# CederGroupHub/sparse-lm

Hardware: AMD Instinct MI355X
Metric: fits/sec over 50-alpha Lasso path at n=100k p=5k (higher is better)
Workload: dtype f64

## Files before the change

### include/slm_engine.h

```cpp
#ifndef SLM_ENGINE_H
#define SLM_ENGINE_H

#include <stddef.h>
#include <stdint.h>

#ifdef __cplusplus
extern "C" {
#endif

#define SLM_ABI_VERSION 24

typedef enum slm_status {
  SLM_OK = 0,
  SLM_ERR_BAD_ARG = 1,
  SLM_ERR_OOM = 2,
  SLM_ERR_HIP = 3,
  SLM_ERR_NO_DEVICE = 4,
  SLM_ERR_COMM = 5,
  SLM_ERR_NOT_CONVERGED = 6,
  SLM_ERR_NON_FINITE = 7,
  SLM_ERR_UNSUPPORTED = 8
} slm_status;

typedef struct slm_engine slm_engine;
// ... 36 lines not shown
  int32_t route;
  int32_t n_lanes;
  int32_t lane_out;
  int32_t probe_lanes;
  int32_t xtr_only;
} slm_gradient_opts;
int slm_gradient_ex(slm_dataset* ds, const double* z, const slm_gradient_opts* opts, double* g_out, double* loss_out,
                    int32_t reps, double* ms_out);

int slm_gradient_lanes(slm_dataset* ds, int32_t route, int32_t n_lanes, const double* Z, const double* row_weights,
                       const double* n_eff, const int32_t* cov_index, int64_t n_rows, double* G_out, double* loss_out,
                       char* kernels_out, int32_t kernels_len);

#define SLM_WSL_GATHER_X 1u
#define SLM_WSL_XTY 2u
typedef struct slm_ws_lanes_opts {
  int32_t route;
  int32_t n_lanes;
  const double* Z;
  const int32_t* on_ws;
  const double* row_weights;
  const double* n_eff;
  const int32_t* cov_index;
  const int32_t* cols;
  const int32_t* k_end;
  int32_t n_builds;
  uint32_t flags;
} slm_ws_lanes_opts;
int slm_working_set_lanes(slm_dataset* ds, const slm_ws_lanes_opts* opts, double* G_out, double* loss_out, int32_t* set_of_out,
                          int32_t* n_sets_out, double* gram_out, double* xw_out, double* xty_out, char* kernels_out,
// ... 262 lines not shown
```

### sparse-lm_amd/csrc/engine_internal.hpp

```cpp
#pragma once
#include <hip/hip_runtime.h>

#include <dlfcn.h>
#include <stdarg.h>
#include <stdio.h>
#include <stdlib.h>
#include <string.h>

#include <algorithm>
#include <cmath>
#include <chrono>
#include <condition_variable>
#include <memory>
#include <mutex>
#include <numeric>
#include <string>
#include <vector>

#include "../../include/slm_engine.h"
#include "host_logic.hpp"
#include "data_kernels.hpp"
#include "grad_kernel.hpp"
#include "tail_kernels.hpp"
#include "ws_kernels.hpp"
// ... 280 lines not shown
int enqueue_gradient_split(const slm_host::Knobs& kn, slm_dataset* ds, const LaneSetup& ls, const double* y, const int* done, const PathCtl* ctl, const WsArgs* wa,
                           hipEvent_t ev_start, hipEvent_t ev_stop, int64_t n_rows = 0, bool unit_bracket = false, const int* skip = nullptr,
                           GradNames* names = nullptr);
bool split_usable(const slm_host::Knobs& kn, slm_dataset* ds);
int ensure_xt(const slm_host::Knobs& kn, slm_dataset* ds);
int ensure_x32s(slm_dataset* ds, int64_t n_rows, bool* usable);
void x32_drop(slm_dataset* ds);
int enqueue_sample_f32(slm_dataset* ds, int64_t n_rows, double n_eff, int n_lanes, const int* done, bool* queued);
int check_launch();
void launch_rowdot(const slm_host::Knobs& kn, slm_dataset* ds, const SplitKernel* sk, int nblk, int B, SplitArgs& a, hipStream_t s,
                  const char** name = nullptr);
int enqueue_gradient_cov(slm_dataset* ds, int B, const int* entry_of, const int* done, hipEvent_t ev_start, hipEvent_t ev_stop,
                         const PathCtl* ctl = nullptr, const WsArgs* wa = nullptr, GradNames* names = nullptr);
void launch_tail(const TailArgs& ta, hipStream_t s);
int64_t sketch_rows(int64_t n);
int power_iteration(const slm_host::Knobs& kn, slm_dataset* ds, const LaneSetup& ls_in, double* L_out , int iters, int64_t n_rows = 0);
int estimate_lipschitz(const slm_host::Knobs& kn, slm_dataset* ds, double* L_out, int iters);
int allow_big_lds(const void* fn, int device);
static const int kProfStride = 3;
static const int kPowerItersSolve = 2;
int cov_fingerprints(slm_dataset* ds, const double* const* w, int count, double* out );
int cov_find(const slm_dataset* ds, double fp1, double fp2, double n_eff);
void cov_pending_drop(slm_dataset* ds);
int set_singleton_groups(slm_dataset* ds);
static const int kMgEntries = 8;
bool mg_possible(const slm_host::Knobs& kn, const slm_dataset* ds);
int mg_ensure(const slm_host::Knobs& kn, slm_dataset* ds, const double* w, double n_eff, bool own, double fp1, double fp2, int* entry_out);
void mg_invalidate(slm_dataset* ds);
void mg_free(slm_dataset* ds);
int mg_enqueue_round(slm_dataset* ds, const TailArgs& ta, int n_lanes, int inner_iters, const int* done, int n_sets, const int* entry_of_set,
                     const int* set_of);
// ... 1 lines not shown
```

### sparse-lm_amd/csrc/engine_path.hip

```cpp
#include "engine_internal.hpp"
#include "ws_solve_kernels.hpp"

static int ws_policy(const slm_host::Knobs& kn, const slm_dataset* ds, uint32_t flags) {
  if (ds->max_group > WS_KCAP / 2 || ds->n < 4) return 0;
  if (kn.ws == 0 || (flags & SLM_FLAG_NO_WORKING_SET)) return 0;
  const bool big = (double)ds->n * (double)ds->ld >= 67108864.0;
  return (big || (flags & SLM_FLAG_WORKING_SET) || kn.ws == 1) ? 2 : 1;
}

static bool small_ok(const slm_host::Knobs& kn, const slm_dataset* ds, uint32_t flags) {
  if (!(flags & SLM_FLAG_ON_CHIP)) return false;
  if (flags & (SLM_FLAG_NO_RESTART | SLM_FLAG_PROFILE | SLM_FLAG_FISTA_ONLY | SLM_FLAG_WORKING_SET | SLM_FLAG_NO_WORKING_SET))
    return false;
  if (!kn.on_chip) return false;
  return ds->p <= SM_PMAX && (double)ds->n * (double)ds->ld <= 131072.0 && !row_sharded(ds);
}
static bool split_possible(const slm_dataset* ds) {
  return ds->sk != nullptr && (ds->sk->rowdot != nullptr || !ds->XT_failed);
}
static int max_lanes_for(const slm_host::Knobs& kn, const slm_dataset* ds, uint32_t flags) {
  if (small_ok(kn, ds, flags)) return ds->lane_cap;
  if ((ws_policy(kn, ds, flags) == 2 || (double)ds->n * (double)ds->ld >= 67108864.0) && split_possible(ds)) {
    if (ws_policy(kn, ds, flags) == 2 && !row_sharded(ds) && ds->sk->rowdot != nullptr && !ds->XT_failed)
      return kMaxLanes;
// ... 294 lines not shown
      const int l = first_lane[u];
      const double ne = ls.n_eff[l] > 0 ? ls.n_eff[l] : (double)ds->n_global;
      entry_of_set[u] = cov_find(ds, fp[2 * u], fp[2 * u + 1], ne);
      cov_on = entry_of_set[u] >= 0;
    }
    if (cov_on) {
      for (int l = 0; l < B; ++l) cov_entry[l] = entry_of_set[uniq_of[l]];
      if (!ds->cov_Z) SLM_TRY(dalloc(&ds->cov_Z, (size_t)ld * SPLIT_RSTRIDE * SPLIT_HALVES));
    }
  }
  return SLM_OK;
}

int PathCall::kept_sketch() {
  if (ds->sketch_valid && !(o.flags & SLM_FLAG_FRESH_L)) return SLM_OK;
  SLM_TRY(power_iteration(kn, ds, default_lanes(ds, 1), nullptr, slm_host::kSketchPowerIters, sketch_rows(ds->n)));
  HIP_TRY(hipMemcpyAsync(ds->lambda + ds->lane_cap, ds->lambda, sizeof(double), hipMemcpyDeviceToDevice, eng->stream));
  ds->sketch_valid = true;
  return SLM_OK;
}

int PathCall::seed_lipschitz() {
  for (int l = 0; l < kMaxCells; ++l) L_factor[l] = 1.0;
  if (o.L > 0.0 || small) {
    for (int l = 0; l < B; ++l) L[l] = o.L > 0.0 ? o.L : 1.0;
  } else {
    const auto t0 = std::chrono::steady_clock::now();
    bool ran = false;
    const bool sketch = ws_policy(kn, ds, o.flags) == 2 && n >= 65536;
    if (sketch && !(ds->L_valid && !(o.flags & SLM_FLAG_FRESH_L) && !any_rw && !custom_scale)) {
      const bool per_lane = any_rw || custom_scale;
      bool bounded = per_lane && !sharded;
// ... 489 lines not shown
  if (shared_path && interleave && mg_handover) hipLaunchKernelGGL(tail_handover_kernel, dim3(1), dim3(64), 0, s, ta);
  else if (shared_path && interleave && use_ws && !ws_late && !sharded && planned_end > 0 && kn.lag_handover)
    hipLaunchKernelGGL(lag_handover_kernel, dim3(1), dim3(64), 0, s, ta, &ds->ws_ctl->builds, &ds->ws_ctl->stale, (int)(planned_end - enq - 1));
  if (sharded) {
    if (use_ws && wa.Gx) {
      hipLaunchKernelGGL(stop_pack_kernel, dim3(1), dim3(64), 0, s, ta.gdone, ds->ctl, B,
                         wa.Gx + (size_t)wa.n_sets * WS_KCAP * WS_KCAP);
    } else {
      hipLaunchKernelGGL(stop_pack_kernel, dim3(1), dim3(64), 0, s, ta.gdone, ds->ctl, B, ds->stop_words);
      if (ws_comm_rc == 0) ws_comm_rc = all_reduce_sum(eng, ds->stop_words, STOP_WORDS);
      hipLaunchKernelGGL(stop_apply_kernel, dim3(1), dim3(64), 0, s, ta.gdone, ds->stop_words);
    }
  }
}

struct WsNames {
  const char* k[8];
  int n = 0;
  void add(const char* name) { if (n < 8) k[n++] = name; }
};
static void ws_enqueue_build(slm_dataset* ds, const WsArgs& wa, const CovSets* cs, bool xty, const int* done, int n_lanes, hipStream_t s,
                             WsNames* names = nullptr) {
  const int64_t n = ds->n;
  if (cs) {
    hipLaunchKernelGGL(ws_gram_cov_kernel, dim3(WS_TILES * WS_TILES, (unsigned)wa.n_sets), dim3(256), 0, s, wa, *cs);
    if (names) names->add("ws_gram_cov_kernel");
    return;
  }
  hipLaunchKernelGGL(ws_gather_kernel, dim3((unsigned)std::min<int64_t>((n + 31) / 32, 1024), WS_KCAP / 32), dim3(256), 0, s, wa);
  if (names) names->add("ws_gather_kernel");
  if (xty) {
    XtyArgs xa;
    xa.ws = wa.ws; xa.idx = wa.idx; xa.XW = wa.XW; xa.y = ds->y; xa.part = wa.part; xa.g = ds->g; xa.gprev = ds->gprev; xa.z = ds->z;
    xa.ctl = ds->ctl; xa.done = done; xa.n = n; xa.ld = ds->ld; xa.inv_n = 1.0 / (double)ds->n_global; xa.n_lanes = n_lanes;
    xa.nblk = (int)std::max<int64_t>(1, std::min<int64_t>(2 * ds->eng->cus, n / 64));
    hipLaunchKernelGGL(ws_xty_partial_kernel, dim3((unsigned)xa.nblk), dim3(512), 0, s, xa);
    hipLaunchKernelGGL(ws_xty_apply_kernel, dim3(WS_KCAP / 128), dim3(512), 0, s, xa);
    if (names) { names->add("ws_xty_partial_kernel"); names->add("ws_xty_apply_kernel"); }
  }
  hipLaunchKernelGGL(ws_gram_kernel, dim3((unsigned)wa.nblk, (unsigned)wa.n_sets, 1), dim3(WS_GRAM_THREADS), 0, s,
                     wa);
  if (wa.Gx)
    (void)hipMemsetAsync(wa.Gx, 0, sizeof(double) * (size_t)wa.n_sets * WS_KCAP * WS_KCAP, s);
  hipLaunchKernelGGL(ws_gram_reduce_kernel, dim3(WS_TILES * WS_TILES, (unsigned)wa.n_sets), dim3(256),
                     0, s, wa);
  if (names) { names->add("ws_gram_kernel"); names->add("ws_gram_reduce_kernel"); }
}

static void ws_enqueue_solvers(const slm_dataset* ds, const TailArgs& ta, const WsArgs& wa, int B, hipStream_t s, WsNames* names = nullptr) {
  if (wa.one_solver && wa.nt) {
  } else if (ds->singleton) {
    hipLaunchKernelGGL((ws_solve_kernel<false, 0>), dim3(B), dim3(WS_THREADS), 0, s, ta, wa);
    if (names) names->add("ws_solve_kernel<false,0>");
// ... 7 lines not shown
    if (names) names->add(ds->singleton ? "ws_solve_kernel<false,1>" : "ws_solve_kernel<true,1>");
  }
}

void PathCall::enqueue_refinement() {
  if (use_ws) {
    {
      const int bs = ds->singleton ? 256 : 64;
      const int64_t items = ds->singleton ? p : 16 * (int64_t)G;
      hipLaunchKernelGGL(ws_score_kernel, dim3((unsigned)((items + bs - 1) / bs)), dim3(bs), 0, s, ta, wa);
      hipLaunchKernelGGL(ws_select_kernel, dim3(1), dim3(WS_THREADS), 0, s, ta, wa);
    }
    if (cov_on) {
      CovSets cs;
      for (int st = 0; st < kMaxLanes; ++st) cs.G[st] = st < wa.n_sets ? ds->cov[(size_t)cov_entry[wa.set_lane[st]]].G : nullptr;
      ws_enqueue_build(ds, wa, &cs, false, done_flag, B, s);
    } else {
      ws_enqueue_build(ds, wa, nullptr, fix_start, done_flag, B, s);
    }
    if (wa.Gx) {
      const size_t gram_words = (size_t)wa.n_sets * WS_KCAP * WS_KCAP;
      if (ws_comm_rc == 0) ws_comm_rc = all_reduce_sum(eng, wa.Gx, gram_words + STOP_WORDS);
      hipLaunchKernelGGL(ws_publish_kernel, dim3(WS_PUBLISH_BLOCKS, (unsigned)wa.n_sets), dim3(256), 0, s, wa);
      hipLaunchKernelGGL(stop_apply_kernel, dim3(1), dim3(64), 0, s, ta.gdone, wa.Gx + gram_words);
    }
    ws_enqueue_solvers(ds, ta, wa, B, s);
  }
}

void PathCall::plan_queue() {
  chunk = o.check_every;
  if (chunk <= 0) {
    const double est_us = std::max(12.0, (double)n * (double)ld * 8.0 / 5.0e6);
// ... 469 lines not shown
  lane.pen = pen;
  lane.points = points;
  lane.n_points = n_points;
  lane.beta0 = beta0;
  lane.betas_out = betas_out;
  lane.group_norms_out = group_norms_out;
  lane.infos = infos;
  return slm_solve_lanes(ds, &lane, 1, opts, stats);
}

extern "C" int slm_working_set_lanes(slm_dataset* ds, const slm_ws_lanes_opts* o, double* G_out, double* loss_out, int32_t* set_of_out,
                                     int32_t* n_sets_out, double* gram_out, double* xw_out, double* xty_out, char* kernels_out,
                                     int32_t kernels_len) {
  if (!ds || !o || !o->Z || !o->cols || !o->k_end || !G_out) return fail(SLM_ERR_BAD_ARG, "NULL argument");
  const int route = o->route, B = o->n_lanes, nb = o->n_builds;
  const bool gather_x = (o->flags & SLM_WSL_GATHER_X) != 0, xty = (o->flags & SLM_WSL_XTY) != 0;
  if (route != 1 && route != 2) return fail(SLM_ERR_BAD_ARG, "route must be 1 (split pass) or 2 (covariance), got %d", route);
  if (B < 1 || B > kMaxLanes) return fail(SLM_ERR_BAD_ARG, "between 1 and %d lanes, got %d", kMaxLanes, B);
  if (o->flags & ~(SLM_WSL_GATHER_X | SLM_WSL_XTY)) return fail(SLM_ERR_BAD_ARG, "unknown flags %#x", o->flags);
  if (xty != (xty_out != nullptr)) return fail(SLM_ERR_BAD_ARG, "xty_out goes with SLM_WSL_XTY");
  if (row_sharded(ds)) return fail(SLM_ERR_UNSUPPORTED, "slm_working_set_lanes: row-sharded datasets");
  if (B > ds->lane_cap) return fail(SLM_ERR_UNSUPPORTED, "%d lanes: the dataset holds %d", B, ds->lane_cap);
  const int64_t n = ds->n, p = ds->p, ld = ds->ld;
  if (nb < 1) return fail(SLM_ERR_BAD_ARG, "at least one build");
  for (int b = 0; b < nb; ++b)
    if (o->k_end[b] <= (b > 0 ? o->k_end[b - 1] : 0) || o->k_end[b] > WS_KCAP)
      return fail(SLM_ERR_BAD_ARG, "k_end must increase from above 0 to at most %d (build %d: %d)", WS_KCAP, b, o->k_end[b]);
  const int kreal = o->k_end[nb - 1];
  const int K = std::max(16, (kreal + 15) & ~15);
  std::vector<int32_t> pos((size_t)ld, -1);
  for (int k = 0; k < kreal; ++k) {
    const int32_t j = o->cols[k];
    if (j < 0 || j >= p) return fail(SLM_ERR_BAD_ARG, "cols[%d] = %d outside [0, %lld)", k, j, (long long)p);
    if (pos[(size_t)j] >= 0) return fail(SLM_ERR_BAD_ARG, "cols[%d] = %d repeats cols[%d]", k, j, pos[(size_t)j]);
    pos[(size_t)j] = k;
// ... 105 lines not shown
    h->Kreal = kr;
    h->K = std::max(16, (kr + 15) & ~15);
    h->k_new = k_old;
    h->building = 1;
    h->valid = 0;
    h->stale = 0;
    h->counter = 0;
    if (b > 0) h->appends += 1;
    else h->builds += 1;
    SLM_TRY(put(ds->ws_idx, h_idx.data(), sizeof(int32_t) * WS_KCAP));
    SLM_TRY(put(ds->ws_gs, h_gs.data(), sizeof(int32_t) * WS_KCAP));
    SLM_TRY(put(ds->ws_gl, h_gl.data(), sizeof(int32_t) * WS_KCAP));
    SLM_TRY(put(ds->ws_pos, h_pos.data(), sizeof(int32_t) * (size_t)ld));
    SLM_TRY(put(ds->ws_ctl, h, sizeof(WsCtl)));
    WsNames wn;
    ws_enqueue_build(ds, wa, route == 2 ? &cs : nullptr, xty, &ds->gctl->done, B, s, &wn);
    for (int u = 0; u < wn.n; ++u) named(wn.k[u]);
    SLM_TRY(check_launch());
    SLM_TRY(get(h, ds->ws_ctl, sizeof(WsCtl)));
    if (h->valid != 1 || h->building != 0 || h->counter != 0)
      return fail(SLM_ERR_HIP, "build %d: the Gram was not published (valid %d, building %d, counter %d)", b, h->valid, h->building,
                  h->counter);
  }
  if (gram_out)
    for (int st = 0; st < n_sets; ++st)
      HIP_TRY(hipMemcpy2DAsync(gram_out + (size_t)st * K * K, sizeof(double) * K, ds->ws_G + (size_t)st * WS_KCAP * WS_KCAP,
                               sizeof(double) * WS_KCAP, sizeof(double) * K, K, hipMemcpyDeviceToHost, s));
  if (xw_out)
    HIP_TRY(hipMemcpy2DAsync(xw_out, sizeof(double) * K, ds->ws_XW, sizeof(double) * WS_KCAP, sizeof(double) * K, n,
                             hipMemcpyDeviceToHost, s));
  if (xty) {
    std::vector<double> g0((size_t)ld + 16);
    SLM_TRY(get(g0.data(), ds->g, sizeof(double) * (size_t)(ld + 16)));
    for (int k = 0; k < kreal; ++k) xty_out[k] = g0[(size_t)o->cols[k]];
    xty_out[kreal] = g0[(size_t)ld];
  }
  HIP_TRY(hipStreamSynchronize(s));
  std::vector<PathCtl> hc((size_t)B);
  memset(hc.data(), 0, sizeof(PathCtl) * (size_t)B);
  for (int l = 0; l < B; ++l) {
    hc[(size_t)l].zsup = (o->on_ws && o->on_ws[l]) ? 1 : 0;
    hc[(size_t)l].zzero = zzero[(size_t)l];
    hc[(size_t)l].tail_pt = -1;
  }
  SLM_TRY(put(ds->ctl, hc.data(), sizeof(PathCtl) * (size_t)B));
  const int slots = SPLIT_LANES * ((B + SPLIT_LANES - 1) / SPLIT_LANES);
  HIP_TRY(hipMemsetAsync(ds->z, 0, sizeof(double) * (size_t)slots * ld, s));
  HIP_TRY(hipMemcpy2DAsync(ds->z, sizeof(double) * ld, o->Z, sizeof(double) * p, sizeof(double) * p, B, hipMemcpyHostToDevice, s));
  GradNames gn;
  if (route == 1) {
// ... 229 lines not shown
```

### sparse-lm_amd/csrc/engine_solve.hip

```cpp
#include "engine_internal.hpp"

#define SLM_GK(W, C, R, B) {W, C, R, B, 0, grad_fused_kernel<W, C, R, B>, "grad_fused_kernel<" #W "," #C "," #R "," #B ">"}
#define SLM_RK(W, C, B, D) {W, C, 1, B, D, grad_ring_kernel<W, C, B, D>, "grad_ring_kernel<" #W "," #C "," #B "," #D ">"}
static const GradKernel kGradRing[] = {
    SLM_RK(8, 1, 1, 3), SLM_RK(8, 2, 1, 3), SLM_RK(8, 3, 1, 3), SLM_RK(8, 4, 1, 3), SLM_RK(8, 5, 1, 2),
    SLM_RK(8, 1, 2, 3), SLM_RK(8, 2, 2, 3), SLM_RK(8, 3, 2, 3), SLM_RK(8, 4, 2, 3), SLM_RK(8, 5, 2, 2),
    SLM_RK(8, 1, 3, 3), SLM_RK(8, 2, 3, 3), SLM_RK(8, 3, 3, 3), SLM_RK(8, 4, 3, 3), SLM_RK(8, 5, 3, 2),
    SLM_RK(8, 1, 4, 3), SLM_RK(8, 2, 4, 3), SLM_RK(8, 3, 4, 3), SLM_RK(8, 4, 4, 3), SLM_RK(8, 5, 4, 2),
    SLM_RK(8, 1, 5, 3), SLM_RK(8, 2, 5, 3), SLM_RK(8, 3, 5, 3), SLM_RK(8, 4, 5, 3),
    SLM_RK(8, 1, 6, 3), SLM_RK(8, 2, 6, 3), SLM_RK(8, 3, 6, 3),
};
static const GradKernel kGradDefault[] = {
    SLM_GK(1, 1, 4, 1), SLM_GK(2, 1, 4, 1), SLM_GK(4, 1, 4, 1), SLM_GK(8, 1, 4, 1), SLM_GK(8, 2, 4, 1),
    SLM_GK(8, 3, 4, 1), SLM_GK(8, 4, 2, 1), SLM_GK(8, 5, 2, 1), SLM_GK(8, 6, 2, 1), SLM_GK(8, 8, 2, 1),
    SLM_GK(8, 10, 1, 1),
    SLM_GK(1, 1, 4, 2), SLM_GK(2, 1, 4, 2), SLM_GK(4, 1, 4, 2), SLM_GK(8, 1, 4, 2), SLM_GK(8, 2, 4, 2),
    SLM_GK(8, 3, 4, 2), SLM_GK(8, 4, 2, 2), SLM_GK(8, 5, 2, 2), SLM_GK(8, 6, 2, 2), SLM_GK(8, 8, 1, 2),
    SLM_GK(1, 1, 4, 3), SLM_GK(2, 1, 4, 3), SLM_GK(4, 1, 4, 3), SLM_GK(8, 1, 4, 3), SLM_GK(8, 2, 4, 3),
    SLM_GK(8, 3, 4, 3), SLM_GK(8, 4, 2, 3), SLM_GK(8, 5, 2, 3), SLM_GK(8, 6, 1, 3),
    SLM_GK(1, 1, 4, 4), SLM_GK(2, 1, 4, 4), SLM_GK(4, 1, 4, 4), SLM_GK(8, 1, 4, 4), SLM_GK(8, 2, 4, 4),
    SLM_GK(8, 3, 2, 4), SLM_GK(8, 4, 2, 4), SLM_GK(8, 5, 1, 4),
};
static const GradKernel kGradExtra[] = {
    SLM_GK(8, 5, 1, 1), SLM_GK(8, 5, 3, 1), SLM_GK(8, 5, 4, 1), SLM_GK(8, 4, 4, 1), SLM_GK(8, 6, 1, 1),
// ... 316 lines not shown
  }
#undef SLM_TAIL_LAUNCH
}

int check_launch() {
  hipError_t e = hipGetLastError();
  if (e != hipSuccess) return fail(SLM_ERR_HIP, "kernel launch failed: %s", hipGetErrorString(e));
  return SLM_OK;
}

static const int kPowerItersQuery = 16;
int64_t sketch_rows(int64_t n) {
  return std::max<int64_t>(1, n / slm_host::kSketchRowDiv);
}

int power_iteration(const slm_host::Knobs& kn, slm_dataset* ds, const LaneSetup& ls_in, double* L_out , int iters, int64_t n_rows) {
  LaneSetup ls = ls_in;
  if (n_rows > 0) {
    for (int l = 0; l < kMaxLanes; ++l) {
      const double ne = ls.n_eff[l] > 0 ? ls.n_eff[l] : (double)ds->n_global;
      ls.n_eff[l] = ne * (double)n_rows / (double)ds->n;
    }
  }
  hipStream_t s = ds->eng->stream;
  if (kn.power_iters > 0) iters = kn.power_iters;
  hipLaunchKernelGGL(power_init_kernel, dim3(ls.B), dim3(TAIL_THREADS), 0, s, ds->z, (int)ds->p, ds->ld);
  for (int k = 0; k < iters; ++k) {
    if (ds->gk[ls.B - 1]) {
      SLM_TRY(enqueue_gradient(ds, ls, ds->yzero, nullptr, nullptr, nullptr, n_rows));
    } else {
      if (!split_usable(kn, ds)) return fail(SLM_ERR_UNSUPPORTED, "no %d-lane kernel for p = %lld", ls.B, (long long)ds->p);
      SLM_TRY(enqueue_gradient_split(kn, ds, ls, ds->yzero, nullptr, nullptr, nullptr, nullptr, nullptr, n_rows));
    }
    PowerArgs pa;
    pa.g = ds->g;
    pa.v = ds->z;
    pa.lambda = ds->lambda;
    pa.p = (int)ds->p;
    pa.ld = ds->ld;
    hipLaunchKernelGGL(power_step_kernel, dim3(ls.B), dim3(TAIL_THREADS), 0, s, pa);
  }
  SLM_TRY(check_launch());
  if (!L_out) return SLM_OK;
  double lam[SLM_MAX_LANES] = {};
  HIP_TRY(hipMemcpyAsync(lam, ds->lambda, sizeof(double) * ls.B, hipMemcpyDeviceToHost, s));
  HIP_TRY(hipStreamSynchronize(s));
  for (int l = 0; l < ls.B; ++l) {
    if (!std::isfinite(lam[l])) return fail(SLM_ERR_NON_FINITE, "power iteration produced a non-finite value");
    double L = lam[l] * 1.08;
    if (!(L > 0.0)) L = (n_rows > 0) ? 0.0 : 1.0;
    L_out[l] = L;
  }
// ... 771 lines not shown
```

### sparse-lm_amd/csrc/host_logic.hpp

```cpp
#pragma once
#include <stddef.h>
#include <math.h>
#include <stdint.h>
#include <stdio.h>
#include <stdlib.h>

#include <algorithm>
#include <utility>
#include <vector>

#if defined(__HIPCC__)
#define SLM_HD __host__ __device__
#else
#define SLM_HD
#endif

namespace slm_host {

struct PoolLedger {
  struct Idle { int dev; size_t bytes; void* block; };
  struct Live { void* block; int dev; size_t bytes; };
  std::vector<Idle> idle;
  std::vector<Live> live;
  size_t idle_bytes = 0;
// ... 156 lines not shown
  int64_t rows;
  int64_t ld32;
};
inline int64_t sample_ld32(int64_t p) { return (p + 3) / 4 * 4; }
inline SamplePlan sample_plan(int64_t n_s, int64_t p, int64_t ld32, int cus) {
  SamplePlan g;
  g.ld32 = ld32;
  (void)p;
  const int64_t quads = ld32 / 4;
  g.xb = (int)std::max<int64_t>(1, (quads + kSampleThreads - 1) / kSampleThreads);
  if (n_s < 1) n_s = 1;
  const int64_t want = std::max<int64_t>(1, (int64_t)kSampleWgsPerCu * std::max(1, cus) / g.xb);
  g.rows = std::max<int64_t>(kSampleMinRows, (n_s + want - 1) / want);
  g.yb = (int)((n_s + g.rows - 1) / g.rows);
  return g;
}

template <typename Entry>
inline int find_by_fingerprint(const std::vector<Entry>& entries, double fp1, double fp2, double n_eff) {
  for (size_t i = 0; i < entries.size(); ++i)
    if (entries[i].fp1 == fp1 && entries[i].fp2 == fp2 && entries[i].n_eff == n_eff) return (int)i;
  return -1;
}

inline void triangle_tile(int t, int* I_out, int* J_out) {
  int I = 0;
  while ((I + 1) * (I + 2) / 2 <= t) ++I;
  *I_out = I;
  *J_out = t - I * (I + 1) / 2;
}
// ... 121 lines not shown
```

### sparse-lm_amd/csrc/tail_kernels.hpp

```cpp
#pragma once
#include <hip/hip_runtime.h>
#include <stdint.h>

#include "../../include/slm_engine.h"
#include "grad_kernel.hpp"
#include "light_ctl.hpp"
#include "tail_logic.hpp"

namespace slm {

constexpr int TAIL_THREADS = 1024;
constexpr int TAIL_WAVES = TAIL_THREADS / 64;

struct PathCtl {
  int32_t point;
  int32_t n_points;
  int32_t iter;
  int32_t max_iter;
  int32_t done;
  int32_t nonfinite;
  int32_t l_bumps;
  int32_t restarts;
  int64_t total_iter;
  double t;
// ... 875 lines not shown
  if (threadIdx.x != 0) return;
  const double n = words[1];
  if (!(n >= 1.0)) return;
  if (n * words[3] != words[2] * words[2]) {
    gdone[4] = 1;
    gdone[0] = 1;
  } else if (words[0] >= n) {
    gdone[0] = 1;
  }
}

struct PowerArgs {
  const double* g;
  double* v;
  double* lambda;
  int p;
  int64_t ld;
};

static __global__ __launch_bounds__(TAIL_THREADS) void power_step_kernel(PowerArgs a) {
  __shared__ double red[1][TAIL_WAVES];
  a.g += (int64_t)blockIdx.x * (a.ld + 16);
  a.v += (int64_t)blockIdx.x * a.ld;
  a.lambda += blockIdx.x;
  double s[1] = {0.0};
  for (int j = threadIdx.x; j < a.p; j += TAIL_THREADS) s[0] = __builtin_fma(a.g[j], a.g[j], s[0]);
  block_sum<1>(s, red);
  const double nrm = sqrt(s[0]);
  const double inv = nrm > 0.0 ? 1.0 / nrm : 0.0;
  for (int j = threadIdx.x; j < a.p; j += TAIL_THREADS) a.v[j] = a.g[j] * inv;
  if (threadIdx.x == 0) a.lambda[0] = nrm;
}

struct SeedArgs {
  PathCtl* ctl;
  const double* lambda;
  int n_lanes;
  double margin;
  double factor[SLM_MAX_LANES];
};
static __global__ void seed_step_kernel(SeedArgs a) {
  const int l = threadIdx.x;
  if (l >= a.n_lanes) return;
  double L0 = a.lambda[0] * a.margin;
  if (L0 <= 0.0) L0 = 1.0;
  const double L = L0 * a.factor[l];
// ... 30 lines not shown
```

### sparse-lm_amd/csrc/ws_kernels.hpp

```cpp
#pragma once
#include <type_traits>
#include <hip/hip_runtime.h>
#include <stdint.h>

#include "tail_kernels.hpp"
#include "newton_kernels.hpp"

namespace slm {

constexpr int WS_KCAP = 512;
constexpr int WS_KLDS = 112;
constexpr int WS_TILES = WS_KCAP / 16;
constexpr int WS_THREADS = 1024;
constexpr int WS_INNER_MAX = 400;
constexpr int WS_BB_ITERS = 14;
constexpr double WS_BB_MAX_STEP = 20.0;
constexpr double WS_INNER_TOL = 0.05;
constexpr int WS_MAX_REPEATS = 6;
constexpr int WS_NEWTON_AFTER = 16;
constexpr int WS_NEWTON_MAX = 256;
constexpr int WS_AFTER_DIRECT = 40;
constexpr double WS_NEWTON_RQ = 0.05;
constexpr int WS_NEWTON_REFUSALS = 4;
constexpr double WS_NEWTON_ENTER = 0.3;
// ... 551 lines not shown
    ws->building = 1;
    ws->valid = 0;
    ws->stale = 0;
    ws->counter = 0;
    if (append) {
      ws->appends += 1;
    } else {
      ws->builds += 1;
      for (int l = 0; l < SLM_MAX_LANES; ++l) ws->Lw[l] = 0.0;
    }
  }
}

static __global__ __launch_bounds__(WS_THREADS) void ws_select_kernel(TailArgs a, WsArgs w) { ws_select_body(a, w); }

static __global__ __launch_bounds__(256) void ws_gather_kernel(WsArgs w) {
  if (!w.ws->building) return;
  const int K = w.ws->K;
  const int k0 = w.ws->k_new + 32 * (int)blockIdx.y;
  if (k0 >= K) return;
  __shared__ double tile[32][33];
  const int tx = threadIdx.x & 31, ty = threadIdx.x >> 5;
  const int64_t row_tiles = (w.n + 31) / 32;
  int jcol[4];
#pragma unroll
  for (int u = 0; u < 4; ++u) {
    const int k = k0 + ty + 8 * u;
    jcol[u] = k < K ? w.idx[k] : -1;
  }
  for (int64_t rt = blockIdx.x; rt < row_tiles; rt += gridDim.x) {
    const int64_t i0 = rt * 32;
    const int64_t i = i0 + tx;
    double v[4];
#pragma unroll
    for (int u = 0; u < 4; ++u) {
      const int j = jcol[u];
      v[u] = (j >= 0 && i < w.n) ? (w.XT ? w.XT[((rt * w.ld + j) << 5) + tx] : w.X[i * w.ld + j]) : 0.0;
    }
    __syncthreads();
#pragma unroll
    for (int u = 0; u < 4; ++u) tile[ty + 8 * u][tx] = v[u];
    __syncthreads();
    for (int ii = ty; ii < 32; ii += 8) {
      const int64_t i = i0 + ii;
      const int k = k0 + tx;
      if (i < w.n && k < K) w.XW[i * WS_KCAP + k] = tile[tx][ii];
    }
  }
}

struct XtyArgs {
  const WsCtl* ws;
  const int32_t* idx;
  const double* XW;
  const double* y;
  double* part;
  double* g;
  double* gprev;
  double* z;
  PathCtl* ctl;
  const int* done;
  int64_t n, ld;
  double inv_n;
  int n_lanes, nblk;
// ... 52 lines not shown
  const int k = threadIdx.x;
  if (k < K) {
    double sum = 0.0;
#pragma unroll
    for (int w = 0; w < 8; ++w) sum += red[w][k];
    out[k] = sum;
  }
  if (k == WS_KCAP - 1) {
    double sum = 0.0;
#pragma unroll
    for (int w = 0; w < 8; ++w) sum += red_yy[w];
    out[WS_KCAP] = sum;
  }
}
static __global__ __launch_bounds__(512) void ws_xty_apply_kernel(XtyArgs a) {
  if (*a.done) return;
  __shared__ double red[4][128];
  __shared__ double ry[512];
  const int K = a.ws->K;
  const int kl = threadIdx.x & 127, q = threadIdx.x >> 7;
  const int k = (int)blockIdx.x * 128 + kl;
  if ((int)blockIdx.x * 128 >= K) return;
  double s[8] = {0, 0, 0, 0, 0, 0, 0, 0};
  if (k < K) {
    int b = q;
    for (; b + 28 < a.nblk; b += 32) {
#pragma unroll
      for (int u = 0; u < 8; ++u) s[u] += a.part[(int64_t)(b + 4 * u) * (WS_KCAP + 1) + k];
    }
    for (; b < a.nblk; b += 4) s[0] += a.part[(int64_t)b * (WS_KCAP + 1) + k];
  }
  red[q][kl] = ((s[0] + s[1]) + (s[2] + s[3])) + ((s[4] + s[5]) + (s[6] + s[7]));
  if (blockIdx.x == 0) ry[threadIdx.x] = (int)threadIdx.x < a.nblk ? a.part[(int64_t)threadIdx.x * (WS_KCAP + 1) + WS_KCAP] : 0.0;
  __syncthreads();
  if (q == 0 && k < K) {
    const int j = a.idx[k];
    if (j >= 0) {
      const double c = -((red[0][kl] + red[1][kl]) + (red[2][kl] + red[3][kl])) * a.inv_n;
      for (int l = 0; l < a.n_lanes; ++l) {
        a.g[(int64_t)l * (a.ld + 16) + j] = c;
        a.gprev[(int64_t)l * a.ld + j] = c;
        a.z[(int64_t)l * a.ld + j] = 0.0;
      }
    }
  }
  if (blockIdx.x == 0) {
    for (int off = 256; off >= 1; off >>= 1) {
      if ((int)threadIdx.x < off) ry[threadIdx.x] += ry[threadIdx.x + off];
      __syncthreads();
    }
    if (threadIdx.x < (unsigned)a.n_lanes) {
      const int l = threadIdx.x;
      const double loss0 = 0.5 * ry[0] * a.inv_n;
// ... 355 lines not shown
```

### sparse-lm_amd/sparselm_amd/_engine.py

```python

from __future__ import annotations

import ctypes as C
import os
import sys
import threading
import weakref

import numpy as np

_LIB_NAME = "libslm_hip.so"
_LIB_DIR = os.path.join(os.path.dirname(os.path.abspath(__file__)), "_lib")

SLM_OK = 0
SLM_ERR_BAD_ARG = 1
SLM_ERR_OOM = 2
SLM_ERR_HIP = 3
SLM_ERR_NO_DEVICE = 4
SLM_ERR_COMM = 5
SLM_ERR_NOT_CONVERGED = 6
SLM_ERR_NON_FINITE = 7
SLM_ERR_UNSUPPORTED = 8

FLAG_NO_RESTART = 1
# ... 90 lines not shown
class NonFiniteError(EngineError):
    """The iterate became non-finite (counterpart of cvxpy's SolverError / 'infeasible')."""


class _PenaltyStruct(C.Structure):
    _fields_ = [("a", C.c_void_p), ("b", C.c_void_p), ("d", C.c_void_p)]


class _GradientOpts(C.Structure):
    _fields_ = [("route", C.c_int32), ("n_lanes", C.c_int32), ("lane_out", C.c_int32), ("probe_lanes", C.c_int32),
                ("xtr_only", C.c_int32)]


WSL_GATHER_X = 1
WSL_XTY = 2


class _WsLanesOpts(C.Structure):
    _fields_ = [("route", C.c_int32), ("n_lanes", C.c_int32), ("Z", C.c_void_p), ("on_ws", C.c_void_p),
                ("row_weights", C.c_void_p), ("n_eff", C.c_void_p), ("cov_index", C.c_void_p), ("cols", C.c_void_p),
                ("k_end", C.c_void_p), ("n_builds", C.c_int32), ("flags", C.c_uint32)]


WMS_DIRECT, WMS_HARD, WMS_INVALID, WMS_BUILDING, WMS_DISABLED, WMS_STALE, WMS_NONFINITE = 1, 2, 4, 8, 16, 32, 64
WMS_COUNTERS = ("refined", "inner_iters", "newton_steps", "newton_fails", "newton_nopd", "newton_factors", "newton_unknowns",
                "hard_next")


class _WsModelOpts(C.Structure):
    _fields_ = [("n_lanes", C.c_int32), ("kreal", C.c_int32), ("cols", C.c_void_p), ("n_sets", C.c_int32), ("flags", C.c_uint32),
# ... 639 lines not shown
        if Z.shape[1] != self.p:
            raise ValueError(f"Z must have {self.p} columns")
        rw = None if row_weights is None else _f64(row_weights, "row_weights", (B, self.n))
        ne = None if n_eff is None else _f64(n_eff, "n_eff", (B,))
        ci = None if cov_index is None else np.ascontiguousarray(cov_index, dtype=np.int32)
        if ci is not None and ci.shape != (B,):
            raise ValueError(f"cov_index has shape {ci.shape}, expected {(B,)}")
        G = np.empty((B, self.p))
        loss = np.empty(B)
        names = C.create_string_buffer(512)
        _check(self._lib.slm_gradient_lanes(self._h, int(route), B, _ptr(Z), _ptr(rw), _ptr(ne), _ptr(ci), int(n_rows),
                                            _ptr(G), _ptr(loss), names, len(names)))
        return G, loss, names.value.decode()

    def working_set_lanes(self, Z, cols, k_end, on_ws=None, row_weights=None, n_eff=None, route: int = 1, cov_index=None,
                          gather_from_x: bool = False, xty: bool = False, want_xw: bool = False):
        import types

        _sync_knobs()
        Z = _f64(np.atleast_2d(Z), "Z")
        B = Z.shape[0]
        if Z.shape[1] != self.p:
            raise ValueError(f"Z must have {self.p} columns")
        cols = np.ascontiguousarray(cols, dtype=np.int32)
        k_end = np.ascontiguousarray(np.atleast_1d(k_end), dtype=np.int32)
        if k_end.size == 0 or cols.size < int(k_end[-1]):
            raise ValueError("cols must hold k_end[-1] feature indices")
        kreal = int(k_end[-1])
        K = max(16, (kreal + 15) // 16 * 16)
        ow = None if on_ws is None else np.ascontiguousarray(np.broadcast_to(np.asarray(on_ws, dtype=np.int32), (B,)))
        rw = None if row_weights is None else _f64(row_weights, "row_weights", (B, self.n))
        ne = None if n_eff is None else _f64(n_eff, "n_eff", (B,))
        ci = None if cov_index is None else np.ascontiguousarray(cov_index, dtype=np.int32)
        if ci is not None and ci.shape != (B,):
            raise ValueError(f"cov_index has shape {ci.shape}, expected {(B,)}")
        opts = _WsLanesOpts(int(route), B, _ptr(Z), _ptr(ow), _ptr(rw), _ptr(ne), _ptr(ci), _ptr(cols), _ptr(k_end),
                            int(k_end.size), (WSL_GATHER_X if gather_from_x else 0) | (WSL_XTY if xty else 0))
        G = np.empty((B, self.p))
        loss = np.empty(B)
        set_of = np.empty(B, dtype=np.int32)
        n_sets = C.c_int32(0)
        gram = np.empty((B, K, K))
        XW = np.empty((self.n, K)) if want_xw else None
        xt = np.empty(kreal + 1) if xty else None
        names = C.create_string_buffer(4096)
        _check(self._lib.slm_working_set_lanes(self._h, C.byref(opts), _ptr(G), _ptr(loss), _ptr(set_of), C.byref(n_sets),
                                               _ptr(gram), _ptr(XW), _ptr(xt), names, len(names)))
        ns = n_sets.value
        return types.SimpleNamespace(G=G, loss=loss, gram=gram[:ns], set_of=set_of, n_sets=ns, K=K, XW=XW,
                                     xty=None if xt is None else xt[:kreal], yy=None if xt is None else float(xt[kreal]),
                                     kernels=names.value.decode())

    def working_set_model_solve(self, cols, gram, zprev, gprev, z, a0, b0, d0, points, tol, mode, set_of=None, Lw=None,
                                direct: bool = True, hard: bool = False, invalid: bool = False, building: bool = False,
                                disabled: bool = False, stale: bool = False, allow_nonfinite: bool = False, repeats=None,
                                last_point=None, last_cols=None, flags: int = 0):
        import types

        _sync_knobs()
        z = _f64(np.atleast_2d(z), "z")
        B = z.shape[0]
        if z.shape[1] != self.p:
            raise ValueError(f"z must have {self.p} columns")
        cols = np.ascontiguousarray(cols, dtype=np.int32).reshape(-1)
        kreal = int(cols.size)
        K = max(16, (kreal + 15) // 16 * 16)
# ... 620 lines not shown
```

Baseline: 17540.

## Fuse X^T y partial sums into working-set gather kernel

When the working set is built with an X^T y fix-up, the gather kernel that copies selected columns into XW now also accumulates per-block partial dot products with y and y^2. This removes the separate ws_xty_partial_kernel pass that re-read the same columns. The apply kernel is retiled to 16 columns per block with 32 partial-row readers so it can reduce more partial blocks. The power iteration also writes the sketch lambda directly into its second slot instead of issuing an extra device-to-device memcpy. In fused mode the gather now covers all K columns instead of only the newly added ones, which may add traffic, and its grid size is capped by the size of the partial buffer.

```diff
diff --git a/include/slm_engine.h b/include/slm_engine.h
--- a/include/slm_engine.h
+++ b/include/slm_engine.h
@@ -74,6 +74,7 @@
 
 #define SLM_WSL_GATHER_X 1u
 #define SLM_WSL_XTY 2u
+#define SLM_WSL_XTY_BUILD 4u
 typedef struct slm_ws_lanes_opts {
   int32_t route;
   int32_t n_lanes;
diff --git a/sparse-lm_amd/csrc/engine_internal.hpp b/sparse-lm_amd/csrc/engine_internal.hpp
--- a/sparse-lm_amd/csrc/engine_internal.hpp
+++ b/sparse-lm_amd/csrc/engine_internal.hpp
@@ -318,7 +318,8 @@
                          const PathCtl* ctl = nullptr, const WsArgs* wa = nullptr, GradNames* names = nullptr);
 void launch_tail(const TailArgs& ta, hipStream_t s);
 int64_t sketch_rows(int64_t n);
-int power_iteration(const slm_host::Knobs& kn, slm_dataset* ds, const LaneSetup& ls_in, double* L_out , int iters, int64_t n_rows = 0);
+int power_iteration(const slm_host::Knobs& kn, slm_dataset* ds, const LaneSetup& ls_in, double* L_out , int iters, int64_t n_rows = 0,
+                    double* keep = nullptr);
 int estimate_lipschitz(const slm_host::Knobs& kn, slm_dataset* ds, double* L_out, int iters);
 int allow_big_lds(const void* fn, int device);
 static const int kProfStride = 3;
diff --git a/sparse-lm_amd/csrc/engine_path.hip b/sparse-lm_amd/csrc/engine_path.hip
--- a/sparse-lm_amd/csrc/engine_path.hip
+++ b/sparse-lm_amd/csrc/engine_path.hip
@@ -332,8 +332,7 @@
 
 int PathCall::kept_sketch() {
   if (ds->sketch_valid && !(o.flags & SLM_FLAG_FRESH_L)) return SLM_OK;
-  SLM_TRY(power_iteration(kn, ds, default_lanes(ds, 1), nullptr, slm_host::kSketchPowerIters, sketch_rows(ds->n)));
-  HIP_TRY(hipMemcpyAsync(ds->lambda + ds->lane_cap, ds->lambda, sizeof(double), hipMemcpyDeviceToDevice, eng->stream));
+  SLM_TRY(power_iteration(kn, ds, default_lanes(ds, 1), nullptr, slm_host::kSketchPowerIters, sketch_rows(ds->n), ds->lambda + ds->lane_cap));
   ds->sketch_valid = true;
   return SLM_OK;
 }
@@ -853,12 +852,14 @@
   }
 }
 
+enum WsXty { WS_XTY_NONE = 0, WS_XTY_BUILD = 1, WS_XTY_SEPARATE = 2 };
+static_assert(slm_host::kXtyPartStride == WS_KCAP + 1, "a row of partial sums: every position, then y^2");
 struct WsNames {
   const char* k[8];
   int n = 0;
   void add(const char* name) { if (n < 8) k[n++] = name; }
 };
-static void ws_enqueue_build(slm_dataset* ds, const WsArgs& wa, const CovSets* cs, bool xty, const int* done, int n_lanes, hipStream_t s,
+static void ws_enqueue_build(slm_dataset* ds, const WsArgs& wa, const CovSets* cs, WsXty xty, const int* done, int n_lanes, hipStream_t s,
                              WsNames* names = nullptr) {
   const int64_t n = ds->n;
   if (cs) {
@@ -866,16 +867,24 @@
     if (names) names->add("ws_gram_cov_kernel");
     return;
   }
-  hipLaunchKernelGGL(ws_gather_kernel, dim3((unsigned)std::min<int64_t>((n + 31) / 32, 1024), WS_KCAP / 32), dim3(256), 0, s, wa);
-  if (names) names->add("ws_gather_kernel");
-  if (xty) {
+  const bool fused = xty == WS_XTY_BUILD && wa.XT != nullptr;
+  const int64_t part_doubles = (int64_t)ws_row_blocks(ds, false, 1).most * std::max(1, ds->ws_sets) * WS_KCAP * WS_KCAP;
+  const int gather_rows = fused ? slm_host::xty_part_rows(n, part_doubles) : slm_host::gather_row_blocks(n);
+  if (fused) hipLaunchKernelGGL(ws_gather_xty_kernel, dim3((unsigned)gather_rows, WS_KCAP / 32), dim3(256), 0, s, wa, ds->y, wa.part);
+  else hipLaunchKernelGGL(ws_gather_kernel, dim3((unsigned)gather_rows, WS_KCAP / 32), dim3(256), 0, s, wa);
+  if (names) names->add(fused ? "ws_gather_xty_kernel" : "ws_gather_kernel");
+  if (xty != WS_XTY_NONE) {
     XtyArgs xa;
     xa.ws = wa.ws; xa.idx = wa.idx; xa.XW = wa.XW; xa.y = ds->y; xa.part = wa.part; xa.g = ds->g; xa.gprev = ds->gprev; xa.z = ds->z;
     xa.ctl = ds->ctl; xa.done = done; xa.n = n; xa.ld = ds->ld; xa.inv_n = 1.0 / (double)ds->n_global; xa.n_lanes = n_lanes;
-    xa.nblk = (int)std::max<int64_t>(1, std::min<int64_t>(2 * ds->eng->cus, n / 64));
-    hipLaunchKernelGGL(ws_xty_partial_kernel, dim3((unsigned)xa.nblk), dim3(512), 0, s, xa);
-    hipLaunchKernelGGL(ws_xty_apply_kernel, dim3(WS_KCAP / 128), dim3(512), 0, s, xa);
-    if (names) { names->add("ws_xty_partial_kernel"); names->add("ws_xty_apply_kernel"); }
+    xa.nblk = gather_rows;
+    if (!fused) {
+      xa.nblk = (int)std::max<int64_t>(1, std::min<int64_t>(2 * ds->eng->cus, n / 64));
+      hipLaunchKernelGGL(ws_xty_partial_kernel, dim3((unsigned)xa.nblk), dim3(512), 0, s, xa);
+      if (names) names->add("ws_xty_partial_kernel");
+    }
+    hipLaunchKernelGGL(ws_xty_apply_kernel, dim3(WS_KCAP / 16), dim3(512), 0, s, xa);
+    if (names) names->add("ws_xty_apply_kernel");
   }
   hipLaunchKernelGGL(ws_gram_kernel, dim3((unsigned)wa.nblk, (unsigned)wa.n_sets, 1), dim3(WS_GRAM_THREADS), 0, s,
                      wa);
@@ -913,9 +922,9 @@
     if (cov_on) {
       CovSets cs;
       for (int st = 0; st < kMaxLanes; ++st) cs.G[st] = st < wa.n_sets ? ds->cov[(size_t)cov_entry[wa.set_lane[st]]].G : nullptr;
-      ws_enqueue_build(ds, wa, &cs, false, done_flag, B, s);
+      ws_enqueue_build(ds, wa, &cs, WS_XTY_NONE, done_flag, B, s);
     } else {
-      ws_enqueue_build(ds, wa, nullptr, fix_start, done_flag, B, s);
+      ws_enqueue_build(ds, wa, nullptr, fix_start ? WS_XTY_BUILD : WS_XTY_NONE, done_flag, B, s);
     }
     if (wa.Gx) {
       const size_t gram_words = (size_t)wa.n_sets * WS_KCAP * WS_KCAP;
@@ -1415,11 +1424,13 @@
                                      int32_t kernels_len) {
   if (!ds || !o || !o->Z || !o->cols || !o->k_end || !G_out) return fail(SLM_ERR_BAD_ARG, "NULL argument");
   const int route = o->route, B = o->n_lanes, nb = o->n_builds;
-  const bool gather_x = (o->flags & SLM_WSL_GATHER_X) != 0, xty = (o->flags & SLM_WSL_XTY) != 0;
+  const bool gather_x = (o->flags & SLM_WSL_GATHER_X) != 0, xty = (o->flags & (SLM_WSL_XTY | SLM_WSL_XTY_BUILD)) != 0;
+  const WsXty xty_mode = (o->flags & SLM_WSL_XTY_BUILD) ? WS_XTY_BUILD : xty ? WS_XTY_SEPARATE : WS_XTY_NONE;
   if (route != 1 && route != 2) return fail(SLM_ERR_BAD_ARG, "route must be 1 (split pass) or 2 (covariance), got %d", route);
   if (B < 1 || B > kMaxLanes) return fail(SLM_ERR_BAD_ARG, "between 1 and %d lanes, got %d", kMaxLanes, B);
-  if (o->flags & ~(SLM_WSL_GATHER_X | SLM_WSL_XTY)) return fail(SLM_ERR_BAD_ARG, "unknown flags %#x", o->flags);
-  if (xty != (xty_out != nullptr)) return fail(SLM_ERR_BAD_ARG, "xty_out goes with SLM_WSL_XTY");
+  if (o->flags & ~(SLM_WSL_GATHER_X | SLM_WSL_XTY | SLM_WSL_XTY_BUILD)) return fail(SLM_ERR_BAD_ARG, "unknown flags %#x", o->flags);
+  if ((o->flags & SLM_WSL_XTY) && (o->flags & SLM_WSL_XTY_BUILD)) return fail(SLM_ERR_BAD_ARG, "SLM_WSL_XTY or SLM_WSL_XTY_BUILD, not both");
+  if (xty != (xty_out != nullptr)) return fail(SLM_ERR_BAD_ARG, "xty_out goes with SLM_WSL_XTY / SLM_WSL_XTY_BUILD");
   if (row_sharded(ds)) return fail(SLM_ERR_UNSUPPORTED, "slm_working_set_lanes: row-sharded datasets");
   if (B > ds->lane_cap) return fail(SLM_ERR_UNSUPPORTED, "%d lanes: the dataset holds %d", B, ds->lane_cap);
   const int64_t n = ds->n, p = ds->p, ld = ds->ld;
@@ -1555,7 +1566,7 @@
     SLM_TRY(put(ds->ws_pos, h_pos.data(), sizeof(int32_t) * (size_t)ld));
     SLM_TRY(put(ds->ws_ctl, h, sizeof(WsCtl)));
     WsNames wn;
-    ws_enqueue_build(ds, wa, route == 2 ? &cs : nullptr, xty, &ds->gctl->done, B, s, &wn);
+    ws_enqueue_build(ds, wa, route == 2 ? &cs : nullptr, xty_mode, &ds->gctl->done, B, s, &wn);
     for (int u = 0; u < wn.n; ++u) named(wn.k[u]);
     SLM_TRY(check_launch());
     SLM_TRY(get(h, ds->ws_ctl, sizeof(WsCtl)));
@@ -1575,6 +1586,15 @@
     SLM_TRY(get(g0.data(), ds->g, sizeof(double) * (size_t)(ld + 16)));
     for (int k = 0; k < kreal; ++k) xty_out[k] = g0[(size_t)o->cols[k]];
     xty_out[kreal] = g0[(size_t)ld];
+    if (o->flags & SLM_WSL_XTY_BUILD) {
+      int64_t touched = 0;
+      for (int64_t j = 0; j < ld + 16; ++j) {
+        uint64_t bits;
+        memcpy(&bits, &g0[(size_t)j], sizeof(bits));
+        if (j != ld && !(j < ld && pos[(size_t)j] >= 0) && bits != ~0ull) ++touched;
+      }
+      xty_out[kreal + 1] = (double)touched;
+    }
   }
   HIP_TRY(hipStreamSynchronize(s));
   std::vector<PathCtl> hc((size_t)B);
diff --git a/sparse-lm_amd/csrc/engine_solve.hip b/sparse-lm_amd/csrc/engine_solve.hip
--- a/sparse-lm_amd/csrc/engine_solve.hip
+++ b/sparse-lm_amd/csrc/engine_solve.hip
@@ -354,7 +354,8 @@
   return std::max<int64_t>(1, n / slm_host::kSketchRowDiv);
 }
 
-int power_iteration(const slm_host::Knobs& kn, slm_dataset* ds, const LaneSetup& ls_in, double* L_out , int iters, int64_t n_rows) {
+int power_iteration(const slm_host::Knobs& kn, slm_dataset* ds, const LaneSetup& ls_in, double* L_out , int iters, int64_t n_rows,
+                    double* keep) {
   LaneSetup ls = ls_in;
   if (n_rows > 0) {
     for (int l = 0; l < kMaxLanes; ++l) {
@@ -376,6 +377,7 @@
     pa.g = ds->g;
     pa.v = ds->z;
     pa.lambda = ds->lambda;
+    pa.keep = k + 1 == iters ? keep : nullptr;
     pa.p = (int)ds->p;
     pa.ld = ds->ld;
     hipLaunchKernelGGL(power_step_kernel, dim3(ls.B), dim3(TAIL_THREADS), 0, s, pa);
diff --git a/sparse-lm_amd/csrc/host_logic.hpp b/sparse-lm_amd/csrc/host_logic.hpp
--- a/sparse-lm_amd/csrc/host_logic.hpp
+++ b/sparse-lm_amd/csrc/host_logic.hpp
@@ -194,6 +194,17 @@
   g.rows = std::max<int64_t>(kSampleMinRows, (n_s + want - 1) / want);
   g.yb = (int)((n_s + g.rows - 1) / g.rows);
   return g;
+}
+
+constexpr int kGatherRowBlocks = 1024;
+constexpr int kXtyPartStride = 512 + 1;
+inline int gather_row_blocks(int64_t n) {
+  const int64_t tiles = (std::max<int64_t>(n, 1) + 31) / 32;
+  return (int)std::min<int64_t>(tiles, kGatherRowBlocks);
+}
+inline int xty_part_rows(int64_t n, int64_t part_doubles) {
+  const int64_t fit = std::max<int64_t>(1, part_doubles / kXtyPartStride);
+  return (int)std::min<int64_t>(gather_row_blocks(n), fit);
 }
 
 template <typename Entry>
diff --git a/sparse-lm_amd/csrc/tail_kernels.hpp b/sparse-lm_amd/csrc/tail_kernels.hpp
--- a/sparse-lm_amd/csrc/tail_kernels.hpp
+++ b/sparse-lm_amd/csrc/tail_kernels.hpp
@@ -913,6 +913,7 @@
   const double* g;
   double* v;
   double* lambda;
+  double* keep;
   int p;
   int64_t ld;
 };
@@ -928,7 +929,10 @@
   const double nrm = sqrt(s[0]);
   const double inv = nrm > 0.0 ? 1.0 / nrm : 0.0;
   for (int j = threadIdx.x; j < a.p; j += TAIL_THREADS) a.v[j] = a.g[j] * inv;
-  if (threadIdx.x == 0) a.lambda[0] = nrm;
+  if (threadIdx.x == 0) {
+    a.lambda[0] = nrm;
+    if (a.keep != nullptr && blockIdx.x == 0) a.keep[0] = nrm;
+  }
 }
 
 struct SeedArgs {
diff --git a/sparse-lm_amd/csrc/ws_kernels.hpp b/sparse-lm_amd/csrc/ws_kernels.hpp
--- a/sparse-lm_amd/csrc/ws_kernels.hpp
+++ b/sparse-lm_amd/csrc/ws_kernels.hpp
@@ -589,10 +589,11 @@
 
 static __global__ __launch_bounds__(WS_THREADS) void ws_select_kernel(TailArgs a, WsArgs w) { ws_select_body(a, w); }
 
-static __global__ __launch_bounds__(256) void ws_gather_kernel(WsArgs w) {
+template <bool XTY>
+__device__ __forceinline__ void ws_gather_body(const WsArgs& w, const double* __restrict__ y, double* __restrict__ part) {
   if (!w.ws->building) return;
   const int K = w.ws->K;
-  const int k0 = w.ws->k_new + 32 * (int)blockIdx.y;
+  const int k0 = (XTY ? 0 : w.ws->k_new) + 32 * (int)blockIdx.y;
   if (k0 >= K) return;
   __shared__ double tile[32][33];
   const int tx = threadIdx.x & 31, ty = threadIdx.x >> 5;
@@ -603,14 +604,24 @@
     const int k = k0 + ty + 8 * u;
     jcol[u] = k < K ? w.idx[k] : -1;
   }
+  double acc[4] = {0.0, 0.0, 0.0, 0.0};
+  double yy = 0.0;
+  const bool yy_tile = XTY && blockIdx.y == 0;
   for (int64_t rt = blockIdx.x; rt < row_tiles; rt += gridDim.x) {
     const int64_t i0 = rt * 32;
     const int64_t i = i0 + tx;
     double v[4];
+    double yi = 0.0;
+    if (XTY) yi = i < w.n ? y[i] : 0.0;
 #pragma unroll
     for (int u = 0; u < 4; ++u) {
       const int j = jcol[u];
       v[u] = (j >= 0 && i < w.n) ? (w.XT ? w.XT[((rt * w.ld + j) << 5) + tx] : w.X[i * w.ld + j]) : 0.0;
+    }
+    if (XTY) {
+#pragma unroll
+      for (int u = 0; u < 4; ++u) acc[u] = __builtin_fma(v[u], yi, acc[u]);
+      if (yy_tile) yy = __builtin_fma(yi, yi, yy);
     }
     __syncthreads();
 #pragma unroll
@@ -622,7 +633,26 @@
       if (i < w.n && k < K) w.XW[i * WS_KCAP + k] = tile[tx][ii];
     }
   }
-}
+  if (XTY) {
+#pragma unroll
+    for (int off = 16; off >= 1; off >>= 1) {
+#pragma unroll
+      for (int u = 0; u < 4; ++u) acc[u] += __shfl_xor(acc[u], off, 64);
+      if (yy_tile) yy += __shfl_xor(yy, off, 64);
+    }
+    double* out = part + (int64_t)blockIdx.x * (WS_KCAP + 1);
+    if (tx == 0) {
+#pragma unroll
+      for (int u = 0; u < 4; ++u) {
+        const int k = k0 + ty + 8 * u;
+        if (k < K) out[k] = acc[u];
+      }
+      if (yy_tile && ty == 0) out[WS_KCAP] = yy;
+    }
+  }
+}
+static __global__ __launch_bounds__(256) void ws_gather_kernel(WsArgs w) { ws_gather_body<false>(w, nullptr, nullptr); }
+static __global__ __launch_bounds__(256) void ws_gather_xty_kernel(WsArgs w, const double* y, double* part) { ws_gather_body<true>(w, y, part); }
 
 struct XtyArgs {
   const WsCtl* ws;
@@ -705,29 +735,36 @@
   }
 }
 static __global__ __launch_bounds__(512) void ws_xty_apply_kernel(XtyArgs a) {
-  if (*a.done) return;
-  __shared__ double red[4][128];
+  if (*a.done || !a.ws->building) return;
+  __shared__ double red[32][17];
   __shared__ double ry[512];
   const int K = a.ws->K;
-  const int kl = threadIdx.x & 127, q = threadIdx.x >> 7;
-  const int k = (int)blockIdx.x * 128 + kl;
-  if ((int)blockIdx.x * 128 >= K) return;
+  const int kl = threadIdx.x & 15, q = threadIdx.x >> 4;
+  const int k = (int)blockIdx.x * 16 + kl;
+  if ((int)blockIdx.x * 16 >= K) return;
   double s[8] = {0, 0, 0, 0, 0, 0, 0, 0};
   if (k < K) {
     int b = q;
-    for (; b + 28 < a.nblk; b += 32) {
-#pragma unroll
-      for (int u = 0; u < 8; ++u) s[u] += a.part[(int64_t)(b + 4 * u) * (WS_KCAP + 1) + k];
-    }
-    for (; b < a.nblk; b += 4) s[0] += a.part[(int64_t)b * (WS_KCAP + 1) + k];
+    for (; b + 224 < a.nblk; b += 256) {
+#pragma unroll
+      for (int u = 0; u < 8; ++u) s[u] += a.part[(int64_t)(b + 32 * u) * (WS_KCAP + 1) + k];
+    }
+    for (; b < a.nblk; b += 32) s[0] += a.part[(int64_t)b * (WS_KCAP + 1) + k];
   }
   red[q][kl] = ((s[0] + s[1]) + (s[2] + s[3])) + ((s[4] + s[5]) + (s[6] + s[7]));
-  if (blockIdx.x == 0) ry[threadIdx.x] = (int)threadIdx.x < a.nblk ? a.part[(int64_t)threadIdx.x * (WS_KCAP + 1) + WS_KCAP] : 0.0;
+  if (blockIdx.x == 0) {
+    double t = 0.0;
+    for (int b = threadIdx.x; b < a.nblk; b += 512) t += a.part[(int64_t)b * (WS_KCAP + 1) + WS_KCAP];
+    ry[threadIdx.x] = t;
+  }
   __syncthreads();
   if (q == 0 && k < K) {
     const int j = a.idx[k];
     if (j >= 0) {
-      const double c = -((red[0][kl] + red[1][kl]) + (red[2][kl] + red[3][kl])) * a.inv_n;
+      double t = 0.0;
+#pragma unroll
+      for (int w = 0; w < 32; ++w) t += red[w][kl];
+      const double c = -t * a.inv_n;
       for (int l = 0; l < a.n_lanes; ++l) {
         a.g[(int64_t)l * (a.ld + 16) + j] = c;
         a.gprev[(int64_t)l * a.ld + j] = c;
diff --git a/sparse-lm_amd/sparselm_amd/_engine.py b/sparse-lm_amd/sparselm_amd/_engine.py
--- a/sparse-lm_amd/sparselm_amd/_engine.py
+++ b/sparse-lm_amd/sparselm_amd/_engine.py
@@ -128,6 +128,7 @@
 
 WSL_GATHER_X = 1
 WSL_XTY = 2
+WSL_XTY_BUILD = 4
 
 
 class _WsLanesOpts(C.Structure):
@@ -797,7 +798,7 @@
         return G, loss, names.value.decode()
 
     def working_set_lanes(self, Z, cols, k_end, on_ws=None, row_weights=None, n_eff=None, route: int = 1, cov_index=None,
-                          gather_from_x: bool = False, xty: bool = False, want_xw: bool = False):
+                          gather_from_x: bool = False, xty: bool = False, want_xw: bool = False, xty_build: bool = False):
         import types
 
         _sync_knobs()
@@ -818,21 +819,28 @@
         if ci is not None and ci.shape != (B,):
             raise ValueError(f"cov_index has shape {ci.shape}, expected {(B,)}")
         opts = _WsLanesOpts(int(route), B, _ptr(Z), _ptr(ow), _ptr(rw), _ptr(ne), _ptr(ci), _ptr(cols), _ptr(k_end),
-                            int(k_end.size), (WSL_GATHER_X if gather_from_x else 0) | (WSL_XTY if xty else 0))
+                            int(k_end.size), (WSL_GATHER_X if gather_from_x else 0) | (WSL_XTY if xty else 0) |
+                            (WSL_XTY_BUILD if xty_build else 0))
         G = np.empty((B, self.p))
         loss = np.empty(B)
         set_of = np.empty(B, dtype=np.int32)
         n_sets = C.c_int32(0)
         gram = np.empty((B, K, K))
         XW = np.empty((self.n, K)) if want_xw else None
-        xt = np.empty(kreal + 1) if xty else None
+        xt = np.empty(kreal + 2) if (xty or xty_build) else None
         names = C.create_string_buffer(4096)
         _check(self._lib.slm_working_set_lanes(self._h, C.byref(opts), _ptr(G), _ptr(loss), _ptr(set_of), C.byref(n_sets),
                                                _ptr(gram), _ptr(XW), _ptr(xt), names, len(names)))
         ns = n_sets.value
         return types.SimpleNamespace(G=G, loss=loss, gram=gram[:ns], set_of=set_of, n_sets=ns, K=K, XW=XW,
                                      xty=None if xt is None else xt[:kreal], yy=None if xt is None else float(xt[kreal]),
-                                     kernels=names.value.decode())
+                                     touched_outside=int(xt[kreal + 1]) if xty_build else None, kernels=names.value.decode())
+
+    def ws_build(self, cols, k_end=None, xty: bool = False, gather_from_x: bool = False, want_xw: bool = False):
+        cols = np.ascontiguousarray(cols, dtype=np.int32)
+        r = self.working_set_lanes(np.zeros((1, self.p)), cols, [cols.size] if k_end is None else k_end, on_ws=[0],
+                                   gather_from_x=gather_from_x, want_xw=want_xw, xty_build=xty)
+        return r
 
     def working_set_model_solve(self, cols, gram, zprev, gprev, z, a0, b0, d0, points, tol, mode, set_of=None, Lw=None,
                                 direct: bool = True, hard: bool = False, invalid: bool = False, building: bool = False,
```

Result: faster. 17730 (median of 6 runs) (+1.1%).
